# jyegerlehner/tensorflow-wavenet

Measured on AMD Instinct MI355X. Metric: audio samples/sec (train, default wavenet_params.json), higher is better.
Workload: dtype f32

## Files before the change

include/wavenet_hip.h:

```cpp
#ifndef WAVENET_HIP_H_
#define WAVENET_HIP_H_

#include <stdint.h>

#ifdef __cplusplus
extern "C" {
#endif

#define WN_OK 0
#define WN_ERR_BAD_SHAPE (-1)
#define WN_ERR_UNSUPPORTED (-2)
#define WN_ERR_MISALIGNED (-3)
#define WN_ERR_LAUNCH (-4)
#define WN_ERR_NULL (-5)

int wn_version(void);
const char* wn_error_string(int code);

int wn_mu_law_thresholds_host(int Q, float* thr_out);
int wn_mu_law_decode_table_host(int Q, float* lut_out);
int wn_mu_law_encode(const float* audio, int32_t* codes, long n,
                     const float* thr_dev, int Q, void* stream);
int wn_mu_law_decode(const int32_t* codes, float* audio, long n,
                     const float* lut_dev, int Q, void* stream);
// ... 81 lines not shown
                      const float* bias, long bias_layer_stride,
                      int bias_clip_stride, const int* dilations, unsigned* flags,
                      unsigned* ctl, float* poison, int L, int B, int T, int save_sg,
                      int variant, const float* skip_img, const float* skip_bsum,
                      float* h1, void* stream);
int wn_stack_fwd_lc(float* X, float* Z, float* SG, const float* wimg,
                    const float* bias, long bias_layer_stride,
                    int bias_clip_stride, const int* dilations, unsigned* flags,
                    unsigned* ctl, float* poison, int L, int B, int T, int save_sg,
                    int variant, const float* lc_add, long lc_row_stride,
                    void* stream);
int wn_stack_bwd_slabs(int B, int T, int variant);
int wn_stack_fwd_waves(int B, int T, int variant);
int wn_stack_bwd_waves(int B, int T, int variant, int* tiles_per_wave);
int wn_stack_bwd(const float* X, const float* Z, const float* SG,
                 const float* dZ, float* DX, long dx_layer_stride, float* Q,
                 const float* wimg, float* slabs,
                 long slab_layer_stride, float* tilesum, const int* dilations,
                 unsigned* flags, unsigned* ctl, float* poison, int L, int B,
                 int T, int variant, void* stream);
int wn_stack_bwd_lc(const float* X, const float* Z, const float* SG,
                    const float* dZ, float* DX, long dx_layer_stride, float* Q,
                    const float* wimg, float* slabs,
                    long slab_layer_stride, float* tilesum, const int* dilations,
                    unsigned* flags, unsigned* ctl, float* poison, int L, int B,
                    int T, int variant, float* lc_da, long lc_row_stride,
                    void* stream);

int wn_gemm_nn(const float* A, long lda, int a_planes, long a_plane_stride,
               const float* W, int ldw, const float* bias, const float* mask,
               long ld_mask, const float* addend, long ld_add, float* C,
               long ldc, int c_planes, long c_plane_stride, float* Cpre,
               long M, int N, int K, int relu, void* stream);

long wn_gemm_split_w_bytes(int K, int N);
int wn_gemm_nn_split(const float* A, long lda, int a_planes,
                     long a_plane_stride, const float* W, int ldw,
                     const float* bias, const float* mask, long ld_mask,
                     const float* addend, long ld_add, float* C, long ldc,
                     int c_planes, long c_plane_stride, float* Cpre, long M,
                     int N, int K, int relu, void* w_scratch, int nprod,
                     void* stream);
long wn_gemm_tn_slab_floats(int Mw, int Nw);
int wn_gemm_tn_tail_rows(int Mw, int Nw);
int wn_gemm_tn_splits(long rows, int Mw, int Nw, int kind);
int wn_gemm_tn_split(const float* A, long lda, int a_planes,
                     long a_plane_stride, const float* G, long ldg,
                     float* slabs, int splits, long rows, int Mw, int Nw,
                     int want_colsum, int nprod, void* stream);
int wn_gemm_tn(const float* A, long lda, int a_planes, long a_plane_stride,
               const int32_t* codes, int shift, int T, const float* G,
               long ldg, float* slabs, int splits, long rows, int Mw, int Nw,
               int want_colsum, void* stream);
int wn_reduce_slabs(const float* slabs, int num_slabs, long slab_stride,
                    int batch, long in_batch_stride, long offset, long n,
                    float* dst, long out_batch_stride, int replicate,
                    long rep_stride, void* stream);
int wn_reduce_slabs_mt(const float* slabs, int num_slabs, long slab_stride,
                       long n_main, float* dst_main, long n_tail, float* dst_tail,
                       int replicate, long rep_stride, int tail_rows, void* stream);
int wn_reduce_pair_slabs(const float* slabs, int num_slabs, int CB, int K,
                         int has_dense, int use_bias, float* layer_grad, int C,
                         long off_bias, int tap0, int Ktot, void* stream);
int wn_transpose(const float* in, int rows, int cols, long in_ld, float* out,
                 long out_ld, void* stream);

int wn_xent_partials(long rows);
int wn_xent(const float* logits, long ld, const int32_t* q, float* dlogits,
            float* loss_partials, int B, int T, int Q, int tf_quirk,
            void* stream);
int wn_xent_masked(const float* logits, long ld, const int32_t* q,
                   const int32_t* lengths, const float* inv_den,
                   float* dlogits, float* loss_partials, int B, int T, int Q,
                   int tf_quirk, void* stream);
int wn_softmax64_row(const float* logits_row, int Q, float* proba,
                     void* stream);

int wn_adam(float* p, const float* g, float* m, float* v, long n, float lr_t,
            float beta1, float beta2, float eps, float grad_scale, float l2,
            const float* l2_mask, void* stream);
int wn_momentum(float* p, const float* g, float* acc, long n, float lr,
                float momentum, float grad_scale, float l2,
                const float* l2_mask, void* stream);
int wn_rmsprop(float* p, const float* g, float* ms, float* mom, long n,
               float lr, float decay, float momentum, float eps,
               float grad_scale, float l2, const float* l2_mask,
               void* stream);
int wn_l2_partials_count(void);
int wn_l2_partials(const float* p, long n, const float* mask, float* partials,
                   void* stream);

int wn_gc_bias(const float* layer0, long layer_stride, long off_bias,
               long off_gc, int G, const float* emb, int card,
               const int32_t* ids, float* out, int L, int B, int ch,
               void* stream);
int wn_colsum_clip_chunks(int T);
int wn_colsum_clip(const float* plane0, const float* plane1, int B, int T,
                   float* part, float* out, void* stream);
int wn_gc_grad(const float* layer0, long layer_stride, long off_gc, int G,
               const float* emb, int card, const int32_t* ids,
               const float* dsum, int L, int B, float* glayer0, float* gemb,
               float* scratch , int ch, void* stream);

int wn_causal_conv(const float* x, const float* w, float* y, int B, int T,
                   int Cin, int Cout, int K, int dilation, void* stream);
int wn_time_to_batch(const float* in, float* out, int B, int T, int C,
// ... 204 lines not shown
```

tensorflow-wavenet_amd/csrc/wn_gemm.hip:

```cpp
#include "wn_common.h"
#include <cstdlib>
#include <cstddef>
#include <cstring>

struct GemmNN {
  const float* A;
  long lda;
  long a_plane_stride;
  int a_planes;
  const float* W;
  int ldw;
  const float* bias;
  const float* mask;
  long ld_mask;
  const float* addend;
  long ld_add;
  float* C;
  long ldc;
  long c_plane_stride;
  int c_planes;
  float* Cpre;
  long M;
  int N, K;
  int relu;
// ... 1071 lines not shown
        if (SUM) {
#pragma unroll
          for (int b = 0; b < NF; ++b) keep[s2][b] = bv[s2 & 1][b];
        }
        __builtin_amdgcn_sched_barrier(0);
      }
      if (SUM) {
#pragma unroll
        for (int b = 0; b < NF; ++b) {
          const f32x2 p0 = {keep[0][b], keep[1][b]}, p1 = {keep[2][b], keep[3][b]};
          const f32x2 p2 = {keep[4][b], keep[5][b]}, p3 = {keep[6][b], keep[7][b]};
          cs2[b] += (p0 + p1) + (p2 + p3);
        }
      }
      __builtin_amdgcn_s_setprio(0);
    }
  };
  const bool spread = g.want_colsum == 2;
  const bool do_cs = spread ? true : (g.want_colsum && tm == (split + 3 * tn) % g.tiles_m);
  if (spread) {
    const int own = (tm + split + 3 * tn) % g.tiles_m;
    for (int c0 = 0; c0 < nchunks; c0 += g.tiles_m) {
      const int ce = min(nchunks, c0 + g.tiles_m);
      const int cs_at = min(ce, c0 + own);
      kloop(wn_false{}, c0, cs_at);
      kloop(wn_true{}, cs_at, min(ce, cs_at + 1));
      kloop(wn_false{}, min(ce, cs_at + 1), ce);
    }
  } else if (do_cs) {
    kloop(wn_true{}, 0, nchunks);
  } else {
    kloop(wn_false{}, 0, nchunks);
  }

  float* slab = g.slabs + (long)split * g.slab_stride;
#pragma unroll
  for (int a = 0; a < MF; ++a)
#pragma unroll
    for (int b = 0; b < NF; ++b) {
      const int n = n0 + wave * (NF * 32) + b * 32 + i;
#pragma unroll
      for (int rr = 0; rr < 16; ++rr) {
        const int m = m0 + a * 32 + 8 * (rr >> 2) + 4 * h + (rr & 3);
        __builtin_nontemporal_store(acc[a][b][rr], slab + (long)m * g.Nw + n);
      }
    }
  if (do_cs) {
#pragma unroll
    for (int b = 0; b < NF; ++b) {
      cs[b] += cs2[b].x + cs2[b].y;
      float v = cs[b] + __shfl_xor(cs[b], 32);
      const int n = n0 + wave * (NF * 32) + b * 32 + i;
      if (h == 0) slab[(long)g.Mw * g.Nw + (spread ? (long)tm * g.Nw : 0) + n] = v;
    }
  }
}

template <int NPROD>
__global__ __launch_bounds__(256, 3) void gemm_tn_split_kernel(GemmTN g) {
  constexpr int KR = 16, TT = 128;
  constexpr int STAGE = 2 * KR * TT;
  __shared__ __attribute__((aligned(1024))) float smem[2 * STAGE];
  const int tid = threadIdx.x, lane = tid & 63;
  const int wave = __builtin_amdgcn_readfirstlane(tid >> 6);
  const int i = lane & 31, h = lane >> 5;
  const int wm = wave & 1, wn = wave >> 1;
  const int ntile = gridDim.x;
  const int logical = xcd_remap(blockIdx.x + ntile * blockIdx.y, ntile * gridDim.y);
  const int tile = logical % ntile, split = logical / ntile;
  const int tn = tile % g.tiles_n, tm = tile / g.tiles_n;
  const int m0 = tm * TT, n0 = tn * TT;
  const long r_begin = (long)split * g.rows_per_split;
  long r_end = r_begin + g.rows_per_split;
  if (r_end > g.rows) r_end = g.rows;
  const int nchunks = r_end > r_begin ? (int)((r_end - r_begin) / KR) : 0;

  const int prow = lane >> 5, pcol = (lane & 31) * 4;
  int am = m0 + pcol;
  am = am < g.Mw ? am : g.Mw - 4;
  int gn = n0 + pcol;
  gn = gn < g.Nw ? gn : g.Nw - 4;
  auto stage = [&](int c, int st) {
    float* base = smem + st * STAGE;
    const long r0 = r_begin + (long)c * KR;
#pragma unroll
    for (int q = 0; q < 2; ++q) {
      const int p = wave + 4 * q;
      const long row = r0 + 2 * p + prow;
      const float* src = g.a_planes
                             ? g.A + (long)(am >> 5) * g.a_plane_stride + row * 32 + (am & 31)
                             : g.A + row * g.lda + am;
      __builtin_amdgcn_global_load_lds((gptr_t)src, (lptr_t)(base + p * 256), 16, 0, 0);
      __builtin_amdgcn_global_load_lds((gptr_t)(g.G + row * g.ldg + gn),
                                       (lptr_t)(base + KR * TT + p * 256), 16, 0, 0);
    }
  };

  f32x16 acc[2][2];
#pragma unroll
  for (int a = 0; a < 2; ++a)
#pragma unroll
    for (int b = 0; b < 2; ++b) acc[a][b] = frag_zero();
  float cs[2] = {0.f, 0.f};

  if (nchunks > 0) stage(0, 0);
  for (int c = 0; c < nchunks; ++c) {
// ... 497 lines not shown
      wn_aligned16(G)) {
    int mf2 = 0, nf2 = 0;
    tn_wg_tile(Mw, Nw, &mf2, &nf2);
    if (mf2 && nf2) {
      g.tiles_m = Mw / (mf2 * 32);
      g.tiles_n = Nw / (4 * nf2 * 32);
      dim3 grid2(g.tiles_m * g.tiles_n, splits), block2(256);
      const long rps = (rows + splits - 1) / splits + 96;
      const long a_bytes = (a_planes ? 5 * a_plane_stride + rps * 32 : rps * lda) * 4;
      const bool dma = a_bytes < (1L << 31) && rps * ldg * 4 < (1L << 31);
#define LAUNCH2(mf, nf)                                                          \
  do {                                                                           \
    if (dma) hipLaunchKernelGGL((gemm_tn3_kernel<mf, nf>), grid2, block2, 0, s, g); \
    else hipLaunchKernelGGL((gemm_tn2_kernel<mf, nf>), grid2, block2, 0, s, g);  \
  } while (0)
      if (mf2 == 5 && nf2 == 2) LAUNCH2(5, 2);
      else if (mf2 == 5) LAUNCH2(5, 1);
      else if (nf2 == 2) LAUNCH2(4, 2);
      else LAUNCH2(4, 1);
#undef LAUNCH2
      return wn_check_launch();
    }
  }
  if (want_colsum == 2) return WN_ERR_UNSUPPORTED;
  const int m32 = (Mw + 31) / 32, n32 = (Nw + 31) / 32;
  int NF = (n32 % 2 == 0) ? 2 : 1;
  int MF;
  if (codes) { NF = 1; MF = (m32 % 2 == 0) ? 2 : 1; }
  else if (m32 % 5 == 0) MF = 5;
  else if (m32 % 4 == 0) MF = 4;
  else if (m32 % 2 == 0) MF = 2;
  else MF = 1;
  g.tiles_m = (m32 + MF - 1) / MF;
  g.tiles_n = (n32 + NF - 1) / NF;
  const int wtiles = g.tiles_m * g.tiles_n;
  dim3 grid((wtiles + 3) / 4, splits), block(256);
#define LAUNCH(mf, nf) \
  hipLaunchKernelGGL((gemm_tn_kernel<mf, nf>), grid, block, 0, s, g)
  if (NF == 2) {
    if (MF == 5) LAUNCH(5, 2);
    else if (MF == 4) LAUNCH(4, 2);
    else if (MF == 2) LAUNCH(2, 2);
    else LAUNCH(1, 2);
  } else {
    if (MF == 5) LAUNCH(5, 1);
    else if (MF == 4) LAUNCH(4, 1);
    else if (MF == 2) LAUNCH(2, 1);
    else LAUNCH(1, 1);
  }
#undef LAUNCH
  return wn_check_launch();
}

__global__ __launch_bounds__(64) void reduce_slabs_wave_kernel(
    const float* __restrict__ slabs, int num_slabs, long slab_stride,
    long in_batch_stride, long offset, float* __restrict__ dst,
    long out_batch_stride, int replicate, long rep_stride) {
  const long e = blockIdx.x;
  const int b = blockIdx.y;
  const float* p = slabs + (long)b * in_batch_stride + offset + e;
  float v = 0.f;
  for (int s = threadIdx.x; s < num_slabs; s += 64) v += p[(long)s * slab_stride];
#pragma unroll
  for (int o = 32; o >= 1; o >>= 1) v += __shfl_xor(v, o);
  if (threadIdx.x == 0)
    for (int r = 0; r < replicate; ++r)
      dst[(long)b * out_batch_stride + (long)r * rep_stride + e] = v;
}

int wn_reduce_slabs(const float* slabs, int num_slabs, long slab_stride,
                    int batch, long in_batch_stride, long offset, long n,
                    float* dst, long out_batch_stride, int replicate,
                    long rep_stride, void* stream) {
  if (!slabs || !dst) return WN_ERR_NULL;
  if (num_slabs <= 0 || n <= 0 || batch <= 0 || replicate <= 0)
    return WN_ERR_BAD_SHAPE;
  if (n <= 4 && num_slabs >= 256) {
    hipLaunchKernelGGL(reduce_slabs_wave_kernel, dim3((unsigned)n, batch),
                       dim3(64), 0, (hipStream_t)stream, slabs, num_slabs,
                       slab_stride, in_batch_stride, offset, dst,
                       out_batch_stride, replicate, rep_stride);
    return wn_check_launch();
  }
  if (((n | offset | slab_stride | in_batch_stride | out_batch_stride | rep_stride) & 3) == 0 &&
      wn_aligned16(slabs) && wn_aligned16(dst)) {
    const long n4 = n / 4;
    dim3 grid4((unsigned)((n4 + 63) / 64), batch);
    const bool split = num_slabs >= 32 && (long)grid4.x * batch <= 4096;
    if (split)
      hipLaunchKernelGGL(reduce_slabs4_kernel<4>, grid4, dim3(256), 0, (hipStream_t)stream,
                         slabs, num_slabs, slab_stride, in_batch_stride, offset, n4,
                         dst, out_batch_stride, replicate, rep_stride);
    else
      hipLaunchKernelGGL(reduce_slabs4_kernel<1>, grid4, dim3(64), 0, (hipStream_t)stream,
                         slabs, num_slabs, slab_stride, in_batch_stride, offset, n4,
                         dst, out_batch_stride, replicate, rep_stride);
    return wn_check_launch();
  }
  dim3 grid((unsigned)((n + 255) / 256), batch), block(256);
  hipLaunchKernelGGL(reduce_slabs_kernel, grid, block, 0, (hipStream_t)stream,
                     slabs, num_slabs, slab_stride, in_batch_stride, offset, n,
                     dst, out_batch_stride, replicate, rep_stride);
  return wn_check_launch();
}

int wn_reduce_slabs_mt(const float* slabs, int num_slabs, long slab_stride,
// ... 43 lines not shown
```

tensorflow-wavenet_amd/wavenet/_lib.py:

```python
import ctypes
import os

_HERE = os.path.dirname(os.path.abspath(__file__))
LIB_PATH = os.environ.get('WN_LIB_PATH') or os.path.join(
    os.path.dirname(_HERE), 'libwavenet_hip.so')

c_int, c_long, c_float = ctypes.c_int, ctypes.c_long, ctypes.c_float
c_void_p, c_u64 = ctypes.c_void_p, ctypes.c_uint64
P = c_void_p

SIGNATURES = {
    'wn_version': (c_int, []),
    'wn_error_string': (ctypes.c_char_p, [c_int]),
    'wn_mu_law_thresholds_host': (c_int, [c_int, P]),
    'wn_mu_law_decode_table_host': (c_int, [c_int, P]),
    'wn_mu_law_encode': (c_int, [P, P, c_long, P, c_int, P]),
    'wn_mu_law_decode': (c_int, [P, P, c_long, P, c_int, P]),
    'wn_causal_gather': (c_int, [P, P, P, c_int, c_int, c_int, c_int, c_int,
                                 P]),
    'wn_scalar_causal_fwd': (c_int, [P, P, c_int, P, c_int, c_int, c_int, P]),
    'wn_scalar_causal_wgrad': (c_int, [P, P, P, c_int, c_int, c_int, c_int,
                                       P]),
    'wn_causal_wgrad_slabs': (c_int, [c_long]),
    'wn_causal_wgrad': (c_int, [P, P, P, c_int, c_int, c_int, c_int, P]),
# ... 8 lines not shown
    'wn_stack_fwd_skip': (c_int, [P, P, P, P, P, c_long, c_int, P, P, P, P,
                                  c_int, c_int, c_int, c_int, c_int, P, P, P, P]),
    'wn_stack_fwd_skip_ok': (c_int, [c_int, c_int, c_int, c_int]),
    'wn_stack_skip_img_floats': (c_long, [c_int]),
    'wn_stack_skip_pack': (c_int, [P, c_int, P, P]),
    'wn_stack_fwd_lc': (c_int, [P, P, P, P, P, c_long, c_int, P, P, P, P,
                                c_int, c_int, c_int, c_int, c_int, P, c_long,
                                P]),
    'wn_stack_bwd_slabs': (c_int, [c_int, c_int, c_int]),
    'wn_stack_fwd_waves': (c_int, [c_int, c_int, c_int]),
    'wn_stack_bwd_waves': (c_int, [c_int, c_int, c_int, P]),
    'wn_stack_bwd': (c_int, [P, P, P, P, P, c_long, P, P, P, c_long, P, P, P,
                             P, P, c_int, c_int, c_int, c_int, P]),
    'wn_stack_bwd_lc': (c_int, [P, P, P, P, P, c_long, P, P, P, c_long, P, P,
                                P, P, P, c_int, c_int, c_int, c_int, P, c_long,
                                P]),
    'wn_layer_wgrad_slab_floats': (c_int, []),
    'wn_dense_planes': (c_int, [P, c_long, P, P, P, c_long, P, c_long, c_long, c_int,
                                P]),
    'wn_dense_planes_gate': (c_int, [P, c_long, P, P, c_long, P, P, c_long, P, P,
                                     c_long, c_long, c_int, P]),
    'wn_layer_fwd_k': (c_int, [P, P, P, P, P, P, P, c_int, c_int, c_int, c_int,
                               c_int, c_int, c_int, P]),
    'wn_layer_bwd_k': (c_int, [P, P, P, P, P, P, P, P, P, P, P, c_int, c_int,
                               c_int, c_int, c_int, c_int, c_int, c_long, P]),
    'wn_layer_wgrad_k': (c_int, [P, P, P, P, P, P, c_int, c_int, c_int, c_int,
                                 c_int, c_int, c_int, c_int, c_long, P]),
    'wn_layer_fwd_blk': (c_int, [P, c_long, c_int, P, P, P, P, P, c_int, P, P,
                                 c_int, c_int, c_int, c_int, c_int, c_int,
                                 c_int, P, P, c_long, c_int, c_int, c_int,
                                 c_long, P]),
    'wn_layer_bwd_blk': (c_int, [P, P, c_long, c_int, P, P, P, P, c_int,
                                 c_long, c_int, c_int, c_int, c_int, c_int,
                                 c_int, c_int, c_long, P]),
    'wn_layer_bwd2_slabs': (c_int, [c_int, c_int]),
    'wn_layer_bwd2_wimg_floats': (c_int, []),
    'wn_layer_bwd2_pack': (c_int, [P, c_long, P, c_int, P]),
    'wn_layer_bwd2': (c_int, [P, P, P, P, P, P, P, P, P, P, c_int, c_int,
                              c_int, P]),
    'wn_gemm_nn': (c_int, [P, c_long, c_int, c_long, P, c_int, P, P, c_long,
                           P, c_long, P, c_long, c_int, c_long, P, c_long,
                           c_int, c_int, c_int, P]),
    'wn_gemm_split_w_bytes': (c_long, [c_int, c_int]),
    'wn_gemm_nn_split': (c_int, [P, c_long, c_int, c_long, P, c_int, P, P,
                                 c_long, P, c_long, P, c_long, c_int, c_long,
                                 P, c_long, c_int, c_int, c_int, P, c_int, P]),
    'wn_gemm_tn_tail_rows': (c_int, [c_int, c_int]),
    'wn_gemm_tn_slab_floats': (c_long, [c_int, c_int]),
    'wn_gemm_tn_splits': (c_int, [c_long, c_int, c_int, c_int]),
    'wn_gemm_tn_split': (c_int, [P, c_long, c_int, c_long, P, c_long, P, c_int,
                                 c_long, c_int, c_int, c_int, c_int, P]),
    'wn_gemm_tn': (c_int, [P, c_long, c_int, c_long, P, c_int, c_int, P,
                           c_long, P, c_int, c_long, c_int, c_int, c_int, P]),
    'wn_reduce_slabs': (c_int, [P, c_int, c_long, c_int, c_long, c_long,
                                c_long, P, c_long, c_int, c_long, P]),
    'wn_reduce_slabs_mt': (c_int, [P, c_int, c_long, c_long, P, c_long, P, c_int,
                                   c_long, c_int, P]),
    'wn_reduce_pair_slabs': (c_int, [P, c_int, c_int, c_int, c_int, c_int, P,
                                     c_int, c_long, c_int, c_int, P]),
    'wn_transpose': (c_int, [P, c_int, c_int, c_long, P, c_long, P]),
    'wn_xent_partials': (c_int, [c_long]),
    'wn_xent': (c_int, [P, c_long, P, P, P, c_int, c_int, c_int, c_int, P]),
    'wn_xent_masked': (c_int, [P, c_long, P, P, P, P, P, c_int, c_int, c_int,
                               c_int, P]),
    'wn_softmax64_row': (c_int, [P, c_int, P, P]),
    'wn_adam': (c_int, [P, P, P, P, c_long, c_float, c_float, c_float,
                        c_float, c_float, c_float, P, P]),
    'wn_momentum': (c_int, [P, P, P, c_long, c_float, c_float, c_float,
                            c_float, P, P]),
    'wn_rmsprop': (c_int, [P, P, P, P, c_long, c_float, c_float, c_float,
                           c_float, c_float, c_float, P, P]),
    'wn_l2_partials_count': (c_int, []),
    'wn_l2_partials': (c_int, [P, c_long, P, P, P]),
    'wn_gc_bias': (c_int, [P, c_long, c_long, c_long, c_int, P, c_int, P, P,
                           c_int, c_int, c_int, P]),
    'wn_colsum_clip_chunks': (c_int, [c_int]),
    'wn_colsum_clip': (c_int, [P, P, c_int, c_int, P, P, P]),
    'wn_gc_grad': (c_int, [P, c_long, c_long, c_int, P, c_int, P, P, c_int,
                           c_int, P, P, P, c_int, P]),
    'wn_causal_conv': (c_int, [P, P, P, c_int, c_int, c_int, c_int, c_int,
                               c_int, P]),
    'wn_time_to_batch': (c_int, [P, P, c_int, c_int, c_int, c_int, P]),
    'wn_batch_to_time': (c_int, [P, P, c_int, c_int, c_int, c_int, P]),
    'wn_diag_mfma_peak': (c_int, [P, c_int, c_int, P]),
    'wn_axpy': (c_int, [P, P, c_float, P, c_long, P]),
    'wn_fill': (c_int, [P, c_long, c_float, P]),
    'wn_sum_rows': (c_int, [P, c_int, c_int, P, P]),
    'wn_fastgen_state_floats': (c_long, [P, c_int]),
    'wn_fastgen_init': (c_int, [P, c_long, P, c_int, P]),
    'wn_fastgen_run': (c_int, [P, P, c_long, P, P, P, P, P, P, P, P, c_int,
                               c_int, c_int, P, P, P, c_int, c_int, c_float,
                               c_u64, P, c_int, c_int, c_int, P]),
    'wn_fastgen_run_wide': (c_int, [P, P, c_long, P, P, P, P, P, P, P, P,
                                    c_int, c_int, c_int, c_int, P, P, P, c_int,
                                    c_int, c_float, c_u64, P, c_int, c_int,
                                    c_int, P, P]),
    'wn_fastgen_wide_coop_bytes': (c_long, [c_int, c_int, c_int, c_int]),
    'wn_fastgen_step': (c_int, [P, P, c_long, P, P, P, P, P, P, P, P, c_int,
                                c_int, c_int, P, P, P, P, P, c_int, P, P, P,
                                P, P, P, P]),
    'wn_fastgen_persist_workgroups': (c_int, [c_int, c_int, c_int]),
    'wn_fastgen_persist_role': (c_int, [c_int, c_int, c_int]),
    'wn_fastgen_persist_ll_words': (c_long, [c_int, c_int, c_int]),
    'wn_fastgen_persist': (c_int, [P, P, c_long, P, P, P, P, P, P, P, P, c_int,
                                   c_int, c_int, P, P, P, P, P, c_int, P, P, P,
                                   P, P, P, P, P, c_int, P]),
# ... 166 lines not shown
```

tensorflow-wavenet_amd/wavenet/train_pass.py:

```python
import collections

import torch

from . import _lib
from . import local_condition as lcond
from .workspace import CH

TN_SIDE_SPLIT_FRAC = 0.6

StepPath = collections.namedtuple('StepPath', [
    'fwd', 'save_ts', 'bwd', 'pack_both', 'overlap_tn', 'early_allreduce',
    'causal_wgrad', 'gemm_mode', 'variant'])


def step_path(net, ws, backward, l2=False):
    layers, lc = net._layer_path(), '_lc' if net.Lc else ''
    fwd = layers
    if net.stack_fwd and net._stack_ok():
        skip = (net.stack_fwd_skip and net.gemm_mode == 'fp32' and
                not net.residual_postproc and ws.fwd_skip_ok)
        fwd = 'stack_skip' if skip else 'stack' + lc
    if not backward:
        return StepPath(fwd, 0, None, False, False, False, None,
                        net.gemm_mode, ws.stack_variant)
# ... 240 lines not shown
             L * C, None, None, 0, None, 0, _lib.ptr(ws.dZ), 0, LP,
             N * CH, None, N, L * C, S, 0)
    tns = [('post2', _lib.ptr(ws.h2), S, 0, 0, _lib.ptr(dlog), Q, S, Q,
            _lib.ptr(net._seg(Gr, 'post2_w')),
            _lib.ptr(net._seg(Gr, 'post2_b'))),
           ('post1', _lib.ptr(ws.h1), S, 0, 0, _lib.ptr(ws.dc1), S, S, S,
            _lib.ptr(net._seg(Gr, 'post1_w')),
            _lib.ptr(net._seg(Gr, 'post1_b'))),
           ('skip', _lib.ptr(ws.Z), 0, LP, N * CH, _lib.ptr(ws.dtotal), S,
            L * C, S, _lib.ptr(net._seg(Gr, 'skip_w')),
            _lib.ptr(net._seg(Gr, 'skip_b')), L, S)]
    if not path.overlap_tn:
        nn_seq(net, [nn_dc1, nn_dtotal, nn_dz])
        for key, *a in tns:
            tn(net, ws, path, st, ws.region[key], *a)
        if path.early_allreduce:
            early_allreduce(net)
        return
    nn_seq(net, [nn_dc1, nn_dtotal])
    main_s = torch.cuda.current_stream()
    side_s = side_stream(net)
    _lib.call_py(lambda: (ws.ev_fork.record(main_s),
                          side_s.wait_event(ws.ev_fork)))
    for key, *a in tns:
        tn(net, ws, path, side_s.cuda_stream, ws.region[key + '_side'], *a)
    _lib.call_py(lambda: ws.ev_join.record(side_s))
    nn(net, *(nn_dz + (st,)))


def reduce_slabs(reg, dst, st, count=None, offset=0, n=None, replicate=1,
                 rep_stride=0):
    _lib.call('wn_reduce_slabs', _lib.ptr(reg.buf),
              reg.count if count is None else count, reg.stride, 1, 0, offset,
              reg.n if n is None else n, dst, 0, replicate, rep_stride, st)


def tn(net, ws, path, st, reg, A, lda, a_planes, a_pstride, Gm, ldg, mw, nw,
       dst, dst_bias, replicate=1, rep_stride=0):
    lib = _lib.load()
    N = ws.N
    ub = 1 if net.use_biases else 0
    sp, sl = reg.count, reg.stride
    if path.overlap_tn and 256 < ws.B * ((ws.T + 31) // 32) <= 512:
        sp = max(1, int(sp * TN_SIDE_SPLIT_FRAC))
    mt = bool(ub and dst_bias is not None and (mw * nw) % 4 == 0 and
              nw % 4 == 0 and sl % 4 == 0 and rep_stride % 4 == 0)
    tr = int(lib.wn_gemm_tn_tail_rows(mw, nw)) \
        if mt and path.gemm_mode == 'fp32' else 1
    if path.gemm_mode != 'fp32' and N % 16 == 0:
        sp = min(sp, lib.wn_gemm_tn_splits(N, mw, nw, 2))
        _lib.call('wn_gemm_tn_split', A, lda, a_planes, a_pstride, Gm,
                  ldg, _lib.ptr(reg.buf), sp, N, mw, nw, ub,
                  int(path.gemm_mode[-1]), st)
    else:
        _lib.call_timed('wn_gemm_tn',
                        (A, lda, a_planes, a_pstride, None, 0, ws.T,
                         Gm, ldg, _lib.ptr(reg.buf), sp, N, mw, nw,
                         2 if tr > 1 else ub,
                         st), 2.0 * N * mw * nw, net._gemm_events)
    if mt:
        _lib.call('wn_reduce_slabs_mt', _lib.ptr(reg.buf), sp, sl,
                  mw * nw, dst, nw, dst_bias, replicate, rep_stride,
                  tr, st)
        return
    reduce_slabs(reg, dst, st, sp)
    if ub and dst_bias is not None:
        reduce_slabs(reg, dst_bias, st, sp, offset=mw * nw, n=nw,
                     replicate=replicate, rep_stride=rep_stride)


def bwd_stack(net, ws, path, st):
    B, T, L = ws.B, ws.T, net.L
    tsum = None if ws.dsum is None else \
        ws.tilesum16 if ws.stack_rows == 16 else ws.tilesum
    if not path.pack_both:
        _lib.call('wn_stack_pack', _lib.ptr(net._layer_block(net.params, 0)),
                  net.layer_stride, None, _lib.ptr(ws.wimg_b), L, st)
    bargs = (
        _lib.ptr(ws.X), _lib.ptr(ws.Z),
        _lib.ptr(ws.SG), _lib.ptr(ws.dZ), _lib.ptr(ws.DX),
        ws.N * CH if ws.keep_dx else 0,
        _lib.ptr(ws.DQ), _lib.ptr(ws.wimg_b), _lib.ptr(ws.lslabs),
        ws.lslabs.shape[1] * net.LAYER_BLOCK,
        None if tsum is None else _lib.ptr(tsum),
        _lib.ptr(net._dil_dev), _lib.ptr(ws.stack_flags_b),
        _lib.ptr(ws.stack_ctl_b),
        _lib.ptr(ws.loss_parts[1:]), L, B, T, ws.stack_variant)
    if path.bwd == 'stack_lc':
        _lib.call_timed('wn_stack_bwd_lc', bargs + (
            _lib.ptr(ws.lc_da), L * 64, st), 0.0, net._gemm_events)
    else:
        _lib.call_timed('wn_stack_bwd', bargs + (st,), 0.0,
                        net._gemm_events)
    return ws.DX[0]


def bwd_layer2(net, ws, path, st):
    B, T, L, P = ws.B, ws.T, net.L, net.params
    tsum = None if ws.dsum is None else ws.tilesum
    _lib.call('wn_layer_bwd2_pack', _lib.ptr(net._layer_block(P, 0)),
              net.layer_stride, _lib.ptr(ws.wimg), L, st)
    dxin, xp = None, 0
    for l in range(L - 1, -1, -1):
        dxo = ws.dx[xp]
        _lib.call('wn_layer_bwd2', _lib.ptr(ws.X[l]), _lib.ptr(ws.Z[l]),
                  _lib.ptr(ws.SG[l]), _lib.ptr(ws.dZ[l]),
# ... 112 lines not shown
```

tensorflow-wavenet_amd/wavenet/workspace.py:

```python
import collections

import numpy as np
import torch

from . import _lib
from . import local_condition as lcond

CH = 32

SlabRegion = collections.namedtuple('SlabRegion', 'buf count stride n')


class _Workspace(object):

    def __init__(self, net, B, T, training, parent=None):
        dev = net.device
        L, S, Q = net.L, net.S, net.Q
        CB, CHn = net.CB, net.CHn
        LP = L * CB
        N = B * T
        self.B, self.T, self.N, self.training = B, T, N, training
        self.stack_variant = net._stack_variant_for_launch()
        self.capacity = N if parent is None else parent.capacity
        lib = _lib.load()
        self.fwd_skip_ok = bool(lib.wn_stack_fwd_skip_ok(B, T, S,
                                                         self.stack_variant))

        def alloc(name, shape, dtype=torch.float32, fill=None):
            n = int(np.prod(shape))
            if parent is not None and getattr(parent, name, None) is not None:
                t = getattr(parent, name).reshape(-1)[:n].view(shape)
            else:
                fresh.add(name)
                if fill is None:
                    t = torch.empty(shape, dtype=dtype, device=dev)
                else:
                    t = torch.full(shape, fill, dtype=dtype, device=dev)
            setattr(self, name, t)
            return t

        fresh = set()

        self.plans = {}
        alloc('q', (N,), torch.int32)
        self.gc_ids = alloc('gc_ids', (B,), torch.int32) \
            if net.card is not None else None
        self.audio = alloc('audio', (N,)) if net.scalar_input else None
        alloc('X', (LP, N, CH))
        alloc('Z', (LP, N, CH))
        alloc('h1', (N, S))
        alloc('h2', (N, S))
        alloc('logits', (N, Q))
        alloc('bias_fg', (L, B, 2 * CHn))
        alloc('stack_flags', (lib.wn_stack_flag_count(B, T, L),), torch.int32,
              fill=0)
        alloc('wimg_f', (L, lib.wn_stack_wimg_floats()))
        alloc('stack_ctl', (4,), torch.int32, fill=0)
        if 'stack_ctl' in fresh:
            self.stack_ctl[2] = 1
        alloc('bsum', (S,))
        self.total = alloc('total', (N, S)) if net.residual_postproc else None
        self.nparts = lib.wn_xent_partials(N)
        alloc('loss_parts', (2 + self.nparts,), fill=0.0)
        alloc('loss', (1,), fill=0.0)
        alloc('xent_mask', (B + 1,), torch.int32, fill=0)
        alloc('proba', (Q,))
        lcond.alloc_workspace(net, self, alloc, None)
        if net.blocked:
            alloc('pre', (2 * CB, N, CH))
        if not training:
            return
        self.legacy = net._layer_path() != 'layer'
        self.TH = alloc('TH', (LP, N, CH)) if self.legacy else None
        alloc('SG', (LP, N, CH))
        alloc('dZ', (LP, N, CH))
        alloc('dc1', (N, S))
        alloc('dtotal', (N, S))
        self.dh2 = alloc('dh2', (N, S)) if net.residual_postproc else None
        self.c1 = alloc('c1', (N, S)) if net.residual_postproc else None
        self.da = alloc('da', (2, 2 * CB, N, CH)) if self.legacy else None
        alloc('dx', (2, CB, N, CH))
        self.stack_bwd = bool(net.stack_bwd and net._stack_ok(N))
        if self.stack_bwd:
            self.keep_dx = bool(net.stack_bwd_keep_dx)
            if parent is not None and getattr(parent, 'DX', None) is not None:
                self.keep_dx = parent.keep_dx
            alloc('DX', (L if self.keep_dx else 1, N, CH))
            alloc('DQ', (L, N, CH))
            alloc('wimg_b', (L, lib.wn_stack_wimg_floats()))
            alloc('stack_flags_b', (lib.wn_stack_flag_count(B, T, L),),
                  torch.int32, fill=0)
            alloc('stack_ctl_b', (4,), torch.int32, fill=0)
            if 'stack_ctl_b' in fresh:
                self.stack_ctl_b[2] = 1
        if net.blocked:
            alloc('dzb', (CB, N, CH))
            alloc('wdT', (CHn, CHn))
            alloc('blk_tmp', (max((2 * net.KW + 1) * 1024 + 96, Q * CH,
                                  net.initial_filter_width * CH),))
            alloc('cs_tmp', (B, 64))
        alloc('w2t', (Q, S))
        alloc('w1t', (S, S))
        alloc('wst', (S, L * CHn))
        shared = []

        def region(key, count, stride, n, own=None, side=False):
            if own:
                self.region[key] = SlabRegion(alloc(own, (count, stride)),
                                              count, stride, n)
            else:
                shared.append((key, count, stride, n, side))

        self.region = {}
        ntiles = B * ((T + 31) // 32)
        nslab = max(1, min(512, ntiles // 4))
        alloc('wimg', (L, lib.wn_layer_bwd2_wimg_floats()))
        if net.blocked:
            pair = (2 * min(net.KW, 8) + 1) * 1024 + 96
            nslab = max(1, min(nslab, (8 << 30) // (CB * CB * pair * 4)))
            alloc('pslabs', (CB * CB, nslab, pair))
            self.region['pairs'] = SlabRegion(self.pslabs, nslab, pair, pair)
            alloc('lslabs', (1, 1, 4))
        else:
            counts = dict(
                layers_k=nslab, layers_2=lib.wn_layer_bwd2_slabs(B, T),
                layers_stack=lib.wn_stack_bwd_slabs(B, T, self.stack_variant)
                if self.stack_bwd else 0)
            alloc('lslabs', (L, max(counts.values()), net.LAYER_BLOCK))
            for key, count in counts.items():
                self.region[key] = SlabRegion(
                    self.lslabs, count, net.LAYER_BLOCK,
                    net.LAYER_BLOCK if net.use_biases else net.LAYER_W)
        for key, mw, nw in (('post2', S, Q), ('post1', S, S),
                            ('skip', L * CHn, S)):
            region(key, lib.wn_gemm_tn_splits(N, mw, nw, 0),
                   lib.wn_gemm_tn_slab_floats(mw, nw), mw * nw, side=True)
        sp, K0 = lib.wn_gemm_tn_splits(N, Q, CH, 1), net.initial_filter_width
        region('causal_onehot', sp, lib.wn_gemm_tn_slab_floats(Q, CH), Q * CH)
        region('causal_scalar', sp, K0 * CH, K0 * CH)
        region('causal_segsum', lib.wn_causal_wgrad_slabs(N), 2 * Q * CH,
               2 * Q * CH)
        lcond.alloc_workspace(net, self, alloc, region)
        alloc('slabs', (max(c * s for _, c, s, _, _ in shared),))
        alloc('slabs_tn', (max(c * s for _, c, s, _, sd in shared if sd),))
        for key, count, stride, n, side in shared:
            self.region[key] = SlabRegion(self.slabs[:count * stride], count,
                                          stride, n)
            if side:
                self.region[key + '_side'] = SlabRegion(
                    self.slabs_tn[:count * stride], count, stride, n)
        self.ev_fork = torch.cuda.Event() if dev.type == 'cuda' else None
        self.ev_join = torch.cuda.Event() if dev.type == 'cuda' else None
        self.dsum = alloc('dsum', (L, B, 2 * CHn)) if net.G else None
        self.gc_part = alloc('gc_part', (L, B, net.G)) if net.G else None
        self.stack_rows = lib.wn_stack_tile_rows(B, T, self.stack_variant)
        nt16 = B * ((T + 15) // 16)
        if net.G:
            buf = alloc('tilesum_buf', (L * nt16 * 64,))
            self.tilesum = buf[:L * ntiles * 64].view(L, ntiles, 64)
            self.tilesum16 = buf.view(L, nt16, 64)
        else:
            self.tilesum = self.tilesum16 = None
        self.dsum_part = alloc(
            'dsum_part', (B * lib.wn_colsum_clip_chunks(T) * 64,)) \
            if net.G else None
        alloc('l2_parts', (lib.wn_l2_partials_count(),))
        alloc('l2', (1,), fill=0.0)


def get(net, B, T, training):
    key = (B, T, bool(training))
    ws = net._ws.get(key)
    if ws is not None and training and net._layer_path() != 'layer' \
            and not ws.legacy:
        net._ws = {}
        ws = None
    if ws is not None:
        return ws
    for (b, t, tr), cand in list(net._ws.items()):
        if cand.capacity == cand.N and b == B and B * T <= cand.capacity \
                and (tr or not training):
            ws = _Workspace(net, B, T, training, parent=cand)
            break
    if ws is None:
        prev = [w for (b, t, tr), w in net._ws.items()
                if w.capacity == w.N and tr == bool(training) and b == B]
        t_alloc = T
        if prev and not training:
            t_alloc = max(T, min(2 * max(w.T for w in prev), 1 << 20))
        net._ws = {k: w for k, w in net._ws.items()
                    if w.training != bool(training)}
        owner = _Workspace(net, B, t_alloc, training)
        net._ws[(B, t_alloc, bool(training))] = owner
        ws = owner if t_alloc == T else \
            _Workspace(net, B, T, training, parent=owner)
    net._ws[key] = ws
    if len(net._ws) > 64:
        owners = {k: v for k, v in net._ws.items()
                  if v.capacity == v.N}
        net._ws = owners
        net._ws[key] = ws
    return ws
```

Baseline: 13.56 million.

## Add intra-workgroup K-split TN GEMM kernel for weight-gradient slabs

Adds a TN GEMM kernel where each workgroup holds four K-partitions (1024 threads), each running its own double-buffered LDS pipeline with per-partition wave arrival counters instead of block barriers. The partial accumulators are then reduced through LDS before one slab store. The fp32 post/skip weight-gradient paths use it, which cuts the number of grid splits and so the slab count and reduction traffic. The cost is an LDS-based cross-partition reduction with extra syncs, fewer resident workgroups per CU, and new split-count and workspace sizing logic.

```diff
diff --git a/include/wavenet_hip.h b/include/wavenet_hip.h
--- a/include/wavenet_hip.h
+++ b/include/wavenet_hip.h
@@ -157,6 +157,11 @@
                const int32_t* codes, int shift, int T, const float* G,
                long ldg, float* slabs, int splits, long rows, int Mw, int Nw,
                int want_colsum, void* stream);
+int wn_gemm_tn_kq_splits(long rows, int Mw, int Nw, long lda, int a_planes,
+                         long a_plane_stride, long ldg);
+int wn_gemm_tn_kq(const float* A, long lda, int a_planes, long a_plane_stride,
+                  const float* G, long ldg, float* slabs, int splits, long rows,
+                  int Mw, int Nw, int want_colsum, void* stream);
 int wn_reduce_slabs(const float* slabs, int num_slabs, long slab_stride,
                     int batch, long in_batch_stride, long offset, long n,
                     float* dst, long out_batch_stride, int replicate,
diff --git a/tensorflow-wavenet_amd/csrc/wn_gemm.hip b/tensorflow-wavenet_amd/csrc/wn_gemm.hip
--- a/tensorflow-wavenet_amd/csrc/wn_gemm.hip
+++ b/tensorflow-wavenet_amd/csrc/wn_gemm.hip
@@ -1147,6 +1147,271 @@
       float v = cs[b] + __shfl_xor(cs[b], 32);
       const int n = n0 + wave * (NF * 32) + b * 32 + i;
       if (h == 0) slab[(long)g.Mw * g.Nw + (spread ? (long)tm * g.Nw : 0) + n] = v;
+    }
+  }
+}
+
+template <int MF, int NF, int KQ>
+__global__ __launch_bounds__(256 * KQ) void gemm_tn_kq_kernel(GemmTN g) {
+  constexpr int TM = MF * 32, TNW = 4 * NF * 32, KR = 16;
+  constexpr int STAGE = KR * TM + KR * TNW;
+  constexpr int PA = KR * TM / 256, PG = KR * TNW / 256;
+  constexpr int XACC = MF * NF * 16 * 256;
+  static_assert(XACC + KQ * 4 * NF * 32 <= KQ * 2 * STAGE, "exchange fits the stages");
+  __shared__ __attribute__((aligned(1024))) float smem_all[KQ * 2 * STAGE];
+  __shared__ unsigned arrived[KQ];
+  const int tid = threadIdx.x, lane = tid & 63;
+  const int wave_wg = __builtin_amdgcn_readfirstlane(tid >> 6);
+  const int kq = wave_wg >> 2, wave = wave_wg & 3;
+  const int i = lane & 31, h = lane >> 5;
+  float* smem = smem_all + kq * (2 * STAGE);
+  if (tid < KQ) arrived[tid] = 0u;
+  const int ntile = gridDim.x;
+  const int logical = xcd_remap(blockIdx.x + ntile * blockIdx.y, ntile * gridDim.y);
+  const int tile = logical % ntile, split = logical / ntile;
+  const int tn = tile % g.tiles_n, tm = tile / g.tiles_n;
+  const int m0 = tm * TM, n0 = tn * TNW;
+  const int part = split * KQ + kq;
+  const long r_begin = (long)part * g.rows_per_split;
+  long r_end = r_begin + g.rows_per_split;
+  if (r_end > g.rows) r_end = g.rows;
+  const int nchunks = r_end > r_begin ? (int)((r_end - r_begin + KR - 1) / KR) : 0;
+  const int tail_rows = nchunks ? (int)(r_end - r_begin) - (nchunks - 1) * KR : KR;
+
+  constexpr int NPA = (PA + 3) / 4, NPG = (PG + 3) / 4;
+  const long rowA = g.a_planes ? 32 * 4 : g.lda * 4, rowG = g.ldg * 4;
+  const __amdgpu_buffer_rsrc_t rsA = ep_rsrc(
+      g.a_planes ? g.A + (long)(m0 >> 5) * g.a_plane_stride + r_begin * 32
+                 : g.A + r_begin * g.lda + m0);
+  const __amdgpu_buffer_rsrc_t rsG = ep_rsrc(g.G + r_begin * g.ldg + n0);
+  int voA[3], voG[4];
+  static_assert(NPA <= 3 && NPG <= 4, "pieces per wave");
+#pragma unroll
+  for (int k = 0; k < NPA; ++k) {
+    const int e = (wave + 4 * k) * 256 + lane * 4;
+    const int row = e / TM, col = e - row * TM;
+    voA[k] = g.a_planes ? (int)(((long)(col >> 5) * g.a_plane_stride + row * 32 + (col & 31)) * 4)
+                        : (int)(((long)row * g.lda + col) * 4);
+  }
+#pragma unroll
+  for (int k = 0; k < NPG; ++k) {
+    const int e = (wave + 4 * k) * 256 + lane * 4;
+    const int row = e / TNW, col = e - row * TNW;
+    voG[k] = (int)(((long)row * g.ldg + col) * 4);
+  }
+  auto stage = [&](int c, int st) {
+    float* base = smem + st * STAGE;
+    const long r0 = (long)c * KR;
+    const unsigned sA = (unsigned)(r0 * rowA), sG = (unsigned)(r0 * rowG);
+    float* gb = base + KR * TM;
+    if (tail_rows < KR && c == nchunks - 1) {
+      const f32x4 zero = {0.f, 0.f, 0.f, 0.f};
+#pragma unroll
+      for (int k = 0; k < NPA; ++k)
+        if (wave + 4 * k < PA)
+          *reinterpret_cast<f32x4*>(base + (wave + 4 * k) * 256 + lane * 4) = zero;
+#pragma unroll
+      for (int k = 0; k < NPG; ++k)
+        if (wave + 4 * k < PG)
+          *reinterpret_cast<f32x4*>(gb + (wave + 4 * k) * 256 + lane * 4) = zero;
+      asm volatile("s_waitcnt lgkmcnt(0)" ::: "memory");
+#pragma unroll
+      for (int k = 0; k < NPA; ++k) {
+        const int p = wave + 4 * k;
+        if (p < PA && (p * 256 + lane * 4) / TM < tail_rows)
+          __builtin_amdgcn_raw_ptr_buffer_load_lds(rsA, (lptr_t)(base + p * 256), 16, voA[k], sA, 0, 0);
+      }
+#pragma unroll
+      for (int k = 0; k < NPG; ++k) {
+        const int p = wave + 4 * k;
+        if (p < PG && (p * 256 + lane * 4) / TNW < tail_rows)
+          __builtin_amdgcn_raw_ptr_buffer_load_lds(rsG, (lptr_t)(gb + p * 256), 16, voG[k], sG, 0, 0);
+      }
+      return;
+    }
+#pragma unroll
+    for (int k = 0; k < NPA; ++k) {
+      const int p = wave + 4 * k;
+      if (p < PA)
+        __builtin_amdgcn_raw_ptr_buffer_load_lds(rsA, (lptr_t)(base + p * 256), 16, voA[k], sA, 0, 0);
+    }
+#pragma unroll
+    for (int k = 0; k < NPG; ++k) {
+      const int p = wave + 4 * k;
+      if (p < PG)
+        __builtin_amdgcn_raw_ptr_buffer_load_lds(rsG, (lptr_t)(gb + p * 256), 16, voG[k], sG, 0, 0);
+    }
+  };
+
+  f32x16 acc[MF][NF];
+#pragma unroll
+  for (int a = 0; a < MF; ++a)
+#pragma unroll
+    for (int b = 0; b < NF; ++b) acc[a][b] = frag_zero();
+  float cs[NF];
+  f32x2 cs2[NF];
+#pragma unroll
+  for (int b = 0; b < NF; ++b) {
+    cs[b] = 0.f;
+    cs2[b] = f32x2{0.f, 0.f};
+  }
+
+  __syncthreads();
+  if (nchunks > 0) stage(0, 0);
+  auto kloop = [&](auto cs_tag, int c_begin, int c_end) {
+    constexpr bool SUM = decltype(cs_tag)::value;
+    for (int c = c_begin; c < c_end; ++c) {
+      const int st = c & 1;
+      asm volatile("s_waitcnt vmcnt(0) lgkmcnt(0)" ::: "memory");
+      if (lane == 0)
+        __hip_atomic_fetch_add(&arrived[kq], 1u, __ATOMIC_RELAXED, __HIP_MEMORY_SCOPE_WORKGROUP);
+      const unsigned want = 4u * (unsigned)(c + 1);
+      while ((unsigned)__builtin_amdgcn_readfirstlane((int)__hip_atomic_load(
+                 &arrived[kq], __ATOMIC_RELAXED, __HIP_MEMORY_SCOPE_WORKGROUP)) < want)
+        __builtin_amdgcn_s_sleep(1);
+      asm volatile("" ::: "memory");
+      if (c + 1 < nchunks) stage(c + 1, st ^ 1);
+      const float* al = smem + st * STAGE + h * TM + i;
+      const float* gl = smem + st * STAGE + KR * TM + h * TNW + wave * (NF * 32) + i;
+      __builtin_amdgcn_s_setprio(1);
+      if (SUM && MF * NF == 8) {
+#pragma unroll
+        for (int s2 = 0; s2 < KR / 2; ++s2) {
+          float a_[MF], b_[NF];
+#pragma unroll
+          for (int a = 0; a < MF; ++a) a_[a] = al[2 * s2 * TM + a * 32];
+#pragma unroll
+          for (int b = 0; b < NF; ++b) {
+            b_[b] = gl[2 * s2 * TNW + b * 32];
+            cs[b] += b_[b];
+          }
+#pragma unroll
+          for (int a = 0; a < MF; ++a)
+#pragma unroll
+            for (int b = 0; b < NF; ++b)
+              acc[a][b] = __builtin_amdgcn_mfma_f32_32x32x2f32(a_[a], b_[b], acc[a][b], 0, 0, 0);
+        }
+        __builtin_amdgcn_s_setprio(0);
+        continue;
+      }
+      float av[2][MF], bv[2][NF], keep[KR / 2][NF];
+      static_assert(KR == 16, "column-sum tree");
+      auto fetch = [&](int s2, float (&a_)[MF], float (&b_)[NF]) {
+#pragma unroll
+        for (int a = 0; a < MF; ++a) a_[a] = al[2 * s2 * TM + a * 32];
+#pragma unroll
+        for (int b = 0; b < NF; ++b) b_[b] = gl[2 * s2 * TNW + b * 32];
+      };
+      fetch(0, av[0], bv[0]);
+      __builtin_amdgcn_sched_barrier(0);
+#pragma unroll
+      for (int s2 = 0; s2 < KR / 2; ++s2) {
+        if (s2 + 1 < KR / 2) fetch(s2 + 1, av[(s2 + 1) & 1], bv[(s2 + 1) & 1]);
+        __builtin_amdgcn_sched_barrier(0);
+#pragma unroll
+        for (int a = 0; a < MF; ++a)
+#pragma unroll
+          for (int b = 0; b < NF; ++b)
+            acc[a][b] = __builtin_amdgcn_mfma_f32_32x32x2f32(av[s2 & 1][a], bv[s2 & 1][b],
+                                                             acc[a][b], 0, 0, 0);
+        if (SUM) {
+#pragma unroll
+          for (int b = 0; b < NF; ++b) keep[s2][b] = bv[s2 & 1][b];
+        }
+        __builtin_amdgcn_sched_barrier(0);
+      }
+      if (SUM) {
+#pragma unroll
+        for (int b = 0; b < NF; ++b) {
+          const f32x2 p0 = {keep[0][b], keep[1][b]}, p1 = {keep[2][b], keep[3][b]};
+          const f32x2 p2 = {keep[4][b], keep[5][b]}, p3 = {keep[6][b], keep[7][b]};
+          cs2[b] += (p0 + p1) + (p2 + p3);
+        }
+      }
+      __builtin_amdgcn_s_setprio(0);
+    }
+  };
+  const bool spread = g.want_colsum == 2;
+  const bool do_cs = spread ? true : (g.want_colsum && tm == (split + 3 * tn) % g.tiles_m);
+  if (spread) {
+    const int own = (tm + part + 3 * tn) % g.tiles_m;
+    for (int c0 = 0; c0 < nchunks; c0 += g.tiles_m) {
+      const int ce = min(nchunks, c0 + g.tiles_m);
+      const int cs_at = min(ce, c0 + own);
+      kloop(wn_false{}, c0, cs_at);
+      kloop(wn_true{}, cs_at, min(ce, cs_at + 1));
+      kloop(wn_false{}, min(ce, cs_at + 1), ce);
+    }
+  } else if (do_cs) {
+    kloop(wn_true{}, 0, nchunks);
+  } else {
+    kloop(wn_false{}, 0, nchunks);
+  }
+
+  float* xacc = smem_all + (wave * 64 + lane) * 4;
+  float* xcs = smem_all + XACC;
+  if (do_cs) {
+#pragma unroll
+    for (int b = 0; b < NF; ++b) {
+      cs[b] += cs2[b].x + cs2[b].y;
+      cs[b] += __shfl_xor(cs[b], 32);
+    }
+  }
+  __syncthreads();
+  if (do_cs && h == 0) {
+#pragma unroll
+    for (int b = 0; b < NF; ++b) xcs[((kq * 4 + wave) * NF + b) * 32 + i] = cs[b];
+  }
+#pragma unroll 1
+  for (int q = 1; q < KQ; ++q) {
+    if (kq == q) {
+#pragma unroll
+      for (int a = 0; a < MF; ++a)
+#pragma unroll
+        for (int b = 0; b < NF; ++b)
+#pragma unroll
+          for (int r4 = 0; r4 < 4; ++r4)
+            *reinterpret_cast<f32x4*>(xacc + ((a * NF + b) * 4 + r4) * 1024) =
+                f32x4{acc[a][b][4 * r4], acc[a][b][4 * r4 + 1], acc[a][b][4 * r4 + 2],
+                      acc[a][b][4 * r4 + 3]};
+    }
+    __syncthreads();
+    if (kq == 0) {
+#pragma unroll
+      for (int a = 0; a < MF; ++a)
+#pragma unroll
+        for (int b = 0; b < NF; ++b)
+#pragma unroll
+          for (int r4 = 0; r4 < 4; ++r4) {
+            const f32x4 v = *reinterpret_cast<const f32x4*>(xacc + ((a * NF + b) * 4 + r4) * 1024);
+#pragma unroll
+            for (int e = 0; e < 4; ++e) acc[a][b][4 * r4 + e] += v[e];
+          }
+    }
+    __syncthreads();
+  }
+  if (kq != 0) return;
+
+  float* slab = g.slabs + (long)split * g.slab_stride;
+#pragma unroll
+  for (int a = 0; a < MF; ++a)
+#pragma unroll
+    for (int b = 0; b < NF; ++b) {
+      const int n = n0 + wave * (NF * 32) + b * 32 + i;
+#pragma unroll
+      for (int rr = 0; rr < 16; ++rr) {
+        const int m = m0 + a * 32 + 8 * (rr >> 2) + 4 * h + (rr & 3);
+        __builtin_nontemporal_store(acc[a][b][rr], slab + (long)m * g.Nw + n);
+      }
+    }
+  if (do_cs && h == 0) {
+#pragma unroll
+    for (int b = 0; b < NF; ++b) {
+      float v = cs[b];
+#pragma unroll
+      for (int q = 1; q < KQ; ++q) v += xcs[((q * 4 + wave) * NF + b) * 32 + i];
+      const int n = n0 + wave * (NF * 32) + b * 32 + i;
+      slab[(long)g.Mw * g.Nw + (spread ? (long)tm * g.Nw : 0) + n] = v;
     }
   }
 }
@@ -1750,6 +2015,69 @@
   return wn_check_launch();
 }
 
+#define TN_KQ 4
+static bool tn_kq_tile(int Mw, int Nw, int* mf) {
+  *mf = Mw % 160 == 0 ? 5 : Mw % 128 == 0 ? 4 : 0;
+  return *mf && Nw % 128 == 0;
+}
+
+static long tn_kq_part_rows(long rows, int splits) {
+  const long q = (rows + (long)splits * TN_KQ - 1) / ((long)splits * TN_KQ);
+  return (q + 15) / 16 * 16;
+}
+
+static bool tn_kq_operands_ok(long rows, int splits, long lda, int a_planes,
+                              long a_plane_stride, long ldg) {
+  if ((ldg & 3) || (!a_planes && (lda & 3)) || (a_planes && (a_plane_stride & 3)))
+    return false;
+  const long q = tn_kq_part_rows(rows, splits);
+  const long a_bytes = (a_planes ? 5 * a_plane_stride + q * 32 : q * lda) * 4;
+  return a_bytes < (1L << 31) && q * ldg * 4 < (1L << 31);
+}
+
+int wn_gemm_tn_kq_splits(long rows, int Mw, int Nw, long lda, int a_planes,
+                         long a_plane_stride, long ldg) {
+  int mf = 0;
+  if (rows <= 0 || Mw <= 0 || Nw <= 0 || lda < 0 || ldg <= 0 || !tn_kq_tile(Mw, Nw, &mf))
+    return 0;
+  if (a_planes && Mw != a_planes * 32) return 0;
+  const int tiles = (Mw / (mf * 32)) * (Nw / 128);
+  long s = tn_device_cus() / tiles;
+  if (s > rows / (64 * TN_KQ)) s = rows / (64 * TN_KQ);
+  if (s < 1 || !tn_kq_operands_ok(rows, (int)s, lda, a_planes, a_plane_stride, ldg)) return 0;
+  return (int)s;
+}
+
+int wn_gemm_tn_kq(const float* A, long lda, int a_planes, long a_plane_stride,
+                  const float* G, long ldg, float* slabs, int splits, long rows,
+                  int Mw, int Nw, int want_colsum, void* stream) {
+  if (!A || !G || !slabs) return WN_ERR_NULL;
+  if (rows <= 0 || Mw <= 0 || Nw <= 0 || splits <= 0 || lda < 0 || ldg <= 0 ||
+      want_colsum < 0 || want_colsum > 2)
+    return WN_ERR_BAD_SHAPE;
+  if (a_planes && Mw != a_planes * 32) return WN_ERR_BAD_SHAPE;
+  int mf = 0;
+  if (!tn_kq_tile(Mw, Nw, &mf) ||
+      !tn_kq_operands_ok(rows, splits, lda, a_planes, a_plane_stride, ldg))
+    return WN_ERR_UNSUPPORTED;
+  if (!wn_aligned16(A) || !wn_aligned16(G)) return WN_ERR_MISALIGNED;
+  GemmTN g;
+  g.A = A; g.lda = lda; g.a_plane_stride = a_plane_stride; g.a_planes = a_planes;
+  g.codes = nullptr; g.shift = 0; g.T = 1; g.G = G; g.ldg = ldg;
+  g.slabs = slabs; g.slab_stride = wn_gemm_tn_slab_floats(Mw, Nw);
+  g.rows = rows;
+  g.rows_per_split = tn_kq_part_rows(rows, splits);
+  g.Mw = Mw; g.Nw = Nw; g.want_colsum = want_colsum;
+  g.tiles_m = Mw / (mf * 32);
+  g.tiles_n = Nw / 128;
+  dim3 grid(g.tiles_m * g.tiles_n, splits), block(256 * TN_KQ);
+  if (mf == 5)
+    hipLaunchKernelGGL((gemm_tn_kq_kernel<5, 1, TN_KQ>), grid, block, 0, (hipStream_t)stream, g);
+  else
+    hipLaunchKernelGGL((gemm_tn_kq_kernel<4, 1, TN_KQ>), grid, block, 0, (hipStream_t)stream, g);
+  return wn_check_launch();
+}
+
 __global__ __launch_bounds__(64) void reduce_slabs_wave_kernel(
     const float* __restrict__ slabs, int num_slabs, long slab_stride,
     long in_batch_stride, long offset, float* __restrict__ dst,
diff --git a/tensorflow-wavenet_amd/wavenet/_lib.py b/tensorflow-wavenet_amd/wavenet/_lib.py
--- a/tensorflow-wavenet_amd/wavenet/_lib.py
+++ b/tensorflow-wavenet_amd/wavenet/_lib.py
@@ -84,6 +84,10 @@
                                  c_long, c_int, c_int, c_int, c_int, P]),
     'wn_gemm_tn': (c_int, [P, c_long, c_int, c_long, P, c_int, c_int, P,
                            c_long, P, c_int, c_long, c_int, c_int, c_int, P]),
+    'wn_gemm_tn_kq_splits': (c_int, [c_long, c_int, c_int, c_long, c_int,
+                                     c_long, c_long]),
+    'wn_gemm_tn_kq': (c_int, [P, c_long, c_int, c_long, P, c_long, P, c_int,
+                              c_long, c_int, c_int, c_int, P]),
     'wn_reduce_slabs': (c_int, [P, c_int, c_long, c_int, c_long, c_long,
                                 c_long, P, c_long, c_int, c_long, P]),
     'wn_reduce_slabs_mt': (c_int, [P, c_int, c_long, c_long, P, c_long, P, c_int,
diff --git a/tensorflow-wavenet_amd/wavenet/train_pass.py b/tensorflow-wavenet_amd/wavenet/train_pass.py
--- a/tensorflow-wavenet_amd/wavenet/train_pass.py
+++ b/tensorflow-wavenet_amd/wavenet/train_pass.py
@@ -316,6 +316,12 @@
         _lib.call('wn_gemm_tn_split', A, lda, a_planes, a_pstride, Gm,
                   ldg, _lib.ptr(reg.buf), sp, N, mw, nw, ub,
                   int(path.gemm_mode[-1]), st)
+    elif reg.kq and path.gemm_mode == 'fp32':
+        _lib.call_timed('wn_gemm_tn_kq',
+                        (A, lda, a_planes, a_pstride, Gm, ldg,
+                         _lib.ptr(reg.buf), sp, N, mw, nw,
+                         2 if tr > 1 else ub, st),
+                        2.0 * N * mw * nw, net._gemm_events)
     else:
         _lib.call_timed('wn_gemm_tn',
                         (A, lda, a_planes, a_pstride, None, 0, ws.T,
diff --git a/tensorflow-wavenet_amd/wavenet/workspace.py b/tensorflow-wavenet_amd/wavenet/workspace.py
--- a/tensorflow-wavenet_amd/wavenet/workspace.py
+++ b/tensorflow-wavenet_amd/wavenet/workspace.py
@@ -8,7 +8,14 @@
 
 CH = 32
 
-SlabRegion = collections.namedtuple('SlabRegion', 'buf count stride n')
+SlabRegion = collections.namedtuple('SlabRegion', 'buf count stride n kq',
+                                    defaults=(False,))
+
+
+def tn_splits(lib, gemm_mode, N, mw, nw, lda, a_planes, a_pstride, ldg):
+    sp = lib.wn_gemm_tn_kq_splits(N, mw, nw, lda, a_planes, a_pstride, ldg) \
+        if gemm_mode == 'fp32' else 0
+    return (sp, True) if sp > 0 else (lib.wn_gemm_tn_splits(N, mw, nw, 0), False)
 
 
 class _Workspace(object):
@@ -104,12 +111,12 @@
         alloc('wst', (S, L * CHn))
         shared = []
 
-        def region(key, count, stride, n, own=None, side=False):
+        def region(key, count, stride, n, own=None, side=0, kq=False):
             if own:
                 self.region[key] = SlabRegion(alloc(own, (count, stride)),
                                               count, stride, n)
             else:
-                shared.append((key, count, stride, n, side))
+                shared.append((key, count, stride, n, side, kq))
 
         self.region = {}
         ntiles = B * ((T + 31) // 32)
@@ -131,24 +138,27 @@
                 self.region[key] = SlabRegion(
                     self.lslabs, count, net.LAYER_BLOCK,
                     net.LAYER_BLOCK if net.use_biases else net.LAYER_W)
-        for key, mw, nw in (('post2', S, Q), ('post1', S, S),
-                            ('skip', L * CHn, S)):
-            region(key, lib.wn_gemm_tn_splits(N, mw, nw, 0),
-                   lib.wn_gemm_tn_slab_floats(mw, nw), mw * nw, side=True)
+        for key, mw, nw, lda, planes, pstride in (
+                ('post2', S, Q, S, 0, 0), ('post1', S, S, S, 0, 0),
+                ('skip', L * CHn, S, 0, L * CB, N * CH)):
+            sp, kq = tn_splits(lib, net.gemm_mode, N, mw, nw, lda, planes,
+                               pstride, nw)
+            region(key, sp, lib.wn_gemm_tn_slab_floats(mw, nw), mw * nw,
+                   side=lib.wn_gemm_tn_splits(N, mw, nw, 0), kq=kq)
         sp, K0 = lib.wn_gemm_tn_splits(N, Q, CH, 1), net.initial_filter_width
         region('causal_onehot', sp, lib.wn_gemm_tn_slab_floats(Q, CH), Q * CH)
         region('causal_scalar', sp, K0 * CH, K0 * CH)
         region('causal_segsum', lib.wn_causal_wgrad_slabs(N), 2 * Q * CH,
                2 * Q * CH)
         lcond.alloc_workspace(net, self, alloc, region)
-        alloc('slabs', (max(c * s for _, c, s, _, _ in shared),))
-        alloc('slabs_tn', (max(c * s for _, c, s, _, sd in shared if sd),))
-        for key, count, stride, n, side in shared:
+        alloc('slabs', (max(c * s for _, c, s, _, _, _ in shared),))
+        alloc('slabs_tn', (max(sd * s for _, _, s, _, sd, _ in shared),))
+        for key, count, stride, n, side, kq in shared:
             self.region[key] = SlabRegion(self.slabs[:count * stride], count,
-                                          stride, n)
+                                          stride, n, kq)
             if side:
                 self.region[key + '_side'] = SlabRegion(
-                    self.slabs_tn[:count * stride], count, stride, n)
+                    self.slabs_tn[:side * stride], side, stride, n)
         self.ev_fork = torch.cuda.Event() if dev.type == 'cuda' else None
         self.ev_join = torch.cuda.Event() if dev.type == 'cuda' else None
         self.dsum = alloc('dsum', (L, B, 2 * CHn)) if net.G else None
```

New measurement: 13.29 million. 0.98x the previous value.
